# cv3vpl-lab/cylinder-pose-estimation

Measured on AMD Instinct MI355X. Metric: frames/sec (grid-detect + cylinder fit) on 1920x1200 batch, higher is better.
Workload: dtype f64

## Files before the change

### cylinder-pose-estimation_amd/csrc/ccl.hip

```cpp
#include "cpe_dev.h"

namespace cpe {

namespace {

__device__ __forceinline__ bool pred(const uint8_t *img, size_t i, int thr, int invert)
{
    return (((int)img[i] > thr) ? 1 : 0) != invert;
}

constexpr int CCL_INIT_ROWS = 16;
__global__ __launch_bounds__(256) void k_ccl_init(const uint8_t *__restrict__ img, int rows_total, int h, int w,
                                                  int thr, int invert, const FrameState *__restrict__ st, Window win,
                                                  int *__restrict__ L, int *__restrict__ cnt, CclOutside outside)
{
    const int lane = threadIdx.x & 63;
    for (int rr = 0; rr < CCL_INIT_ROWS / 4; rr++) {
    const int row = (blockIdx.x * (CCL_INIT_ROWS / 4) + rr) * 4 + (threadIdx.x >> 6);
    if (row >= rows_total) return;
    const int f = row / h, y = row - f * h;
    const Rect r = window_rect(st, f, win, h, w);
    if (y < r.y0 || y > r.y1 || r.x1 < r.x0) continue;
    const size_t base = (size_t)row * w;
    int carry_in = 0, carry_start = 0;
// ... 137 lines not shown
        const u64x2 *t = reinterpret_cast<const u64x2 *>(plane + bit_word(tc, y8, x0 >> 6));
#pragma unroll
        for (int q = 0; q < 4; q++) { const u64x2 v = t[q]; m[2 * q] = v.x; m[2 * q + 1] = v.y; }
    }
    __device__ __forceinline__ unsigned colbits(int y8, int ya, int yb, int x) const
    {
        unsigned long long m[CCL_STRIP];
        strip(y8, ya, yb, x & ~63, m);
        unsigned b = 0;
#pragma unroll
        for (int k = 0; k < CCL_STRIP; k++) b |= (unsigned)((m[k] >> (x & 63)) & 1ull) << k;
        return b;
    }
};

struct NotBitSrc {
    BitSrc b;
    size_t frame_words;
    __device__ __forceinline__ NotBitSrc frame(size_t f, int) const
    {
        return NotBitSrc{BitSrc{b.plane + f * frame_words, b.tc, b.plane_words}, frame_words};
    }
    __device__ __forceinline__ unsigned long long pack(int y, int x0) const { return ~b.pack(y, x0); }
    __device__ __forceinline__ bool px(int y, int x) const { return !b.px(y, x); }
    __device__ __forceinline__ void strip(int y8, int ya, int yb, int x0, unsigned long long (&m)[CCL_STRIP]) const
    {
        b.strip(y8, ya, yb, x0, m);
#pragma unroll
        for (int k = 0; k < CCL_STRIP; k++) m[k] = ~m[k];
    }
    __device__ __forceinline__ unsigned colbits(int y8, int ya, int yb, int x) const { return ~b.colbits(y8, ya, yb, x) & 0xffu; }
};

template <class SRC>
__global__ __launch_bounds__(256) void k_ccl_init64(SRC src0, int h, int w,
                                                    const FrameState *__restrict__ st, Window win, int *__restrict__ L)
{
    const int WW = (w + 63) >> 6, strips = (h + CCL_STRIP - 1) / CCL_STRIP;
    const size_t f = blockIdx.y;
    const int gi = blockIdx.x * 256 + threadIdx.x;
    if (gi >= WW * strips) return;
    const int sy = gi / WW, j = gi - sy * WW;
    const Rect r = window_rect(st, f, win, h, w);
    const int x0 = j * 64;
    if (r.x1 < r.x0 || x0 > r.x1 || x0 + 63 < r.x0) return;
    const int ya = max(sy * CCL_STRIP, r.y0), yb = min(sy * CCL_STRIP + CCL_STRIP - 1, r.y1);
    const size_t N = (size_t)h * w;
    const SRC src = src0.frame(f, h);
    int *Lf = L + f * N;
    const unsigned long long cmask = col_mask64(x0, r.x0, r.x1);
    const bool hasL = x0 - 1 >= r.x0;
    const int y8 = sy * CCL_STRIP;
    unsigned long long rows[CCL_STRIP], any = 0;
    src.strip(y8, ya, yb, x0, rows);
#pragma unroll
    for (int k = 0; k < CCL_STRIP; k++) any |= (y8 + k >= ya && y8 + k <= yb) ? rows[k] & cmask : 0ull;
    const unsigned lb = (hasL && (any & 1ull)) ? src.colbits(y8, ya, yb, x0 - 1) : 0u;
#pragma unroll
    for (int k = 0; k < CCL_STRIP; k++) {
        const int y = y8 + k;
        if (y < ya || y > yb) continue;
        unsigned long long m = rows[k] & cmask;
        if (!m) continue;
        const int base = y * w + x0;
        const bool cL = (m & 1ull) && ((lb >> k) & 1u);
        while (m) {
            const unsigned long long low = m & (0ull - m), run = m & ~(m + low);
            const int a = __ffsll((long long)low) - 1, e = a + __popcll(run);
            const int label = (a == 0 && cL) ? base - 1 : base + a;
            int b = a;
            while (b < e) {
                if ((b & 3) == 0 && b + 4 <= e) { *reinterpret_cast<int4 *>(Lf + base + b) = make_int4(label, label, label, label); b += 4; }
                else { Lf[base + b] = label; b++; }
            }
            m &= ~run;
        }
    }
}

template <class SRC>
__global__ __launch_bounds__(256) void k_ccl_merge64(SRC src0, int h, int w,
                                                     int conn8, const FrameState *__restrict__ st, Window win,
                                                     int *__restrict__ L)
{
    const int WW = (w + 63) >> 6, strips = (h + CCL_STRIP - 1) / CCL_STRIP;
    const size_t f = blockIdx.y;
    const int gi = blockIdx.x * 256 + threadIdx.x;
    if (gi >= WW * strips) return;
    const int sy = gi / WW, j = gi - sy * WW;
    const Rect r = window_rect(st, f, win, h, w);
    const int x0 = j * 64;
    if (r.x1 < r.x0 || x0 > r.x1 || x0 + 63 < r.x0) return;
    const int ya = max(sy * CCL_STRIP, r.y0 + 1), yb = min(sy * CCL_STRIP + CCL_STRIP - 1, r.y1);
    if (ya > yb) return;
    const size_t N = (size_t)h * w;
    const SRC src = src0.frame(f, h);
    int *Lf = L + f * N;
    const unsigned long long cmask = col_mask64(x0, r.x0, r.x1);
    const bool hasL = x0 - 1 >= r.x0, hasR = x0 + 64 <= r.x1;
    const int y8 = sy * CCL_STRIP;
    unsigned long long rows[CCL_STRIP], any = 0;
    src.strip(y8, ya - 1, yb, x0, rows);
#pragma unroll
    for (int k = 0; k < CCL_STRIP; k++) any |= (y8 + k >= ya - 1 && y8 + k <= yb) ? rows[k] & cmask : 0ull;
    const unsigned lb = (hasL && (any & 1ull)) ? src.colbits(y8, ya - 1, yb, x0 - 1) : 0u;
    const unsigned rb = (hasR && (any >> 63)) ? src.colbits(y8, ya - 1, yb, x0 + 64) : 0u;
    unsigned long long A = 0, aL = 0, aR = 0;
    if (ya == y8) {
        A = src.pack(ya - 1, x0) & cmask;
        aL = (hasL && src.px(ya - 1, x0 - 1)) ? 1ull : 0ull; aR = (hasR && src.px(ya - 1, x0 + 64)) ? 1ull : 0ull;
    }
#pragma unroll
    for (int k = 0; k < CCL_STRIP; k++) {
        const int y = y8 + k;
        if (y < ya - 1 || y > yb) continue;
        const unsigned long long C = rows[k] & cmask;
        const unsigned long long cL = (lb >> k) & 1u, cR = (rb >> k) & 1u;
        if (y == ya - 1) { A = C; aL = cL; aR = cR; continue; }
        if (C) {
            const unsigned long long Cs = (C << 1) | cL, As = (A << 1) | aL;
            const int base = y * w + x0;
            unsigned long long m = C & A & ~(Cs & As);
            while (m) { const int b = __ffsll((long long)m) - 1; m &= m - 1; uf_unite(Lf, base + b, base + b - w); }
            if (conn8) {
                const unsigned long long Cr = (C >> 1) | (cR << 63), Ar = (A >> 1) | (aR << 63);
                const unsigned long long nu = C & ~A;
                m = nu & Ar & ~Cr;
                while (m) { const int b = __ffsll((long long)m) - 1; m &= m - 1; uf_unite(Lf, base + b, base + b - w + 1); }
                m = nu & As & ~Cs;
                while (m) { const int b = __ffsll((long long)m) - 1; m &= m - 1; uf_unite(Lf, base + b, base + b - w - 1); }
            }
        }
        A = C; aL = cL; aR = cR;
    }
}

template <class SRC>
__global__ __launch_bounds__(256) void k_ccl_roots64(SRC src0, int h, int w,
                                                     FrameState *__restrict__ st, Window win, const int *__restrict__ L,
                                                     int *__restrict__ roots, RootList list)
{
    const int WW = (w + 63) >> 6, strips = (h + CCL_STRIP - 1) / CCL_STRIP;
    const size_t f = blockIdx.y;
    const int lane = threadIdx.x & 63;
    const int gi = blockIdx.x * 256 + threadIdx.x;
    const Rect r = window_rect(st, f, win, h, w);
    const size_t N = (size_t)h * w;
    const SRC src = src0.frame(f, h);
    const int *Lf = L + f * N;
    const int sy = gi / WW, j = gi - sy * WW, x0 = j * 64;
    const bool live = gi < WW * strips && !(r.x1 < r.x0 || x0 > r.x1 || x0 + 63 < r.x0);
    const int ya = live ? max(sy * CCL_STRIP, r.y0) : 0, yb = live ? min(sy * CCL_STRIP + CCL_STRIP - 1, r.y1) : -1;
    const unsigned long long cmask = live ? col_mask64(x0, r.x0, r.x1) : 0ull;
    const bool hasL = live && x0 - 1 >= r.x0;
    const int y8 = sy * CCL_STRIP;
    unsigned long long rows[CCL_STRIP], any = 0;
    unsigned lb = 0;
    if (live) {
        src.strip(y8, ya, yb, x0, rows);
#pragma unroll
        for (int k = 0; k < CCL_STRIP; k++) any |= (y8 + k >= ya && y8 + k <= yb) ? rows[k] & cmask : 0ull;
        if (hasL && (any & 1ull)) lb = src.colbits(y8, ya, yb, x0 - 1);
// ... 544 lines not shown
                if (__ballot(seed != cur)) {
                    o = flood_row(bg, seed, lane, WW);
                    if (lane < WW && o != cur) { out[(size_t)y * WW + lane] = o; any = true; }
                }
                prev = o;
            }
        }
        const int slot = ((pass + 1) >> 1) & 1;
        if (__ballot(any) && lane == 0) atomicOr(&s_any[slot], 1);
        __syncthreads();
        if (!upw) {
            const int ch = s_any[slot];
            __syncthreads();
            if (threadIdx.x == 0) s_any[slot] = 0;
            if (!ch) { converged = true; break; }
        }
    }
    if (!converged && threadIdx.x == 0) set_overflow(st[f], OVF_TRACE);
}

int outside_flood(const uint8_t *mask, int n, int h, int w, FrameState *st, Window win, unsigned long long *bgw,
                  unsigned long long *out, size_t plane_words, hipStream_t s, const uint32_t *bits)
{
    CPE_CHECK_ARG(w <= 4096 && plane_words >= (size_t)h * ((w + 63) >> 6), "outside_flood: frame too wide or scratch too small");
    CPE_LAUNCH_BEGIN();
    CPE_KLAUNCH(k_outside_flood, dim3(n), dim3(64 * FLOOD_BANDS), 0, s, mask, h, w, st, win, bgw, out, plane_words, bits);
    CPE_CHECK_LAUNCH("k_outside_flood");
    return CPE_OK;
}

static bool word_rows(const void *img, const int *L, int w) { return w % 16 == 0 && ((size_t)img & 15) == 0 && ((size_t)L & 15) == 0; }
static dim3 word_grid(int n, int h, int w) { return dim3((unsigned)((((w + 63) / 64) * ((h + CCL_STRIP - 1) / CCL_STRIP) + 255) / 256), n); }

static bool links8(const uint8_t *img, int n, int h, int w, int thr, Window win, int *L, FrameState *st, hipStream_t s)
{
    const size_t N = (size_t)h * w;
    if (word_rows(img, L, w)) {
        const ByteSrc src{img, w, thr, 0};
        CPE_KLAUNCH(k_ccl_init64<ByteSrc>, word_grid(n, h, w), dim3(256), 0, s, src, h, w, (const FrameState *)st, win, L);
        CPE_KLAUNCH(k_ccl_merge64<ByteSrc>, word_grid(n, h, w), dim3(256), 0, s, src, h, w, 1, (const FrameState *)st, win, L);
        return true;
    }
    CPE_KLAUNCH(k_ccl_init, dim3((n * h + CCL_INIT_ROWS - 1) / CCL_INIT_ROWS), dim3(256), 0, s, img, n * h, h, w, thr, 0, (const FrameState *)st, win, L,
                (int *)nullptr, OUTSIDE_UNTOUCHED);
    CPE_KLAUNCH(k_ccl_merge, dim3((unsigned)((N + CCL_BLK_PX - 1) / CCL_BLK_PX), n), dim3(256), 0, s, img, h, w, thr, 0, 1, (const FrameState *)st, win, L);
    return false;
}

bool ccl_components_reads_bits(const uint32_t *bits, int w, const int *L) { return bits && w % 16 == 0 && ((size_t)L & 15) == 0; }

int ccl_components(const uint8_t *img, const uint32_t *bits, int n, int h, int w, int thr, Window win, int *L, int *roots,
                   RootList list, FrameState *st, hipStream_t s)
{
    const size_t N = (size_t)h * w;
    const dim3 gw = word_grid(n, h, w);
    CPE_LAUNCH_BEGIN();
    CPE_KLAUNCH(k_ccl_ctl, dim3((n + 63) / 64), dim3(64), 0, s, st, (int *)nullptr, n, CTL_RESET_ROOTS, list);
    if (ccl_components_reads_bits(bits, w, L)) {
        const BitSrc src{bit_plane(bits, 0, h, w), bit_tile_cols(w), bit_plane_words(h, w)};
        CPE_KLAUNCH(k_ccl_init64<BitSrc>, gw, dim3(256), 0, s, src, h, w, (const FrameState *)st, win, L);
        CPE_KLAUNCH(k_ccl_merge64<BitSrc>, gw, dim3(256), 0, s, src, h, w, 1, (const FrameState *)st, win, L);
        CPE_KLAUNCH(k_ccl_roots64<BitSrc>, gw, dim3(256), 0, s, src, h, w, st, win, (const int *)L, roots, list);
    } else if (links8(img, n, h, w, thr, win, L, st, s)) {
        CPE_KLAUNCH(k_ccl_roots64<ByteSrc>, gw, dim3(256), 0, s, (ByteSrc{img, w, thr, 0}), h, w, st, win, (const int *)L, roots, list);
    } else {
        CPE_KLAUNCH(k_ccl_roots4, dim3((unsigned)((N + CCL_BLK_PX - 1) / CCL_BLK_PX), n), dim3(256), 0, s, img, h, w, thr, 0, st, win, (const int *)L,
                    roots, list);
    }
    CPE_CHECK_LAUNCH("ccl_components");
    return CPE_OK;
}

int ccl_unions(const uint8_t *mask, int n, int h, int w, Window win, int *L, FrameState *st, hipStream_t s)
{
    CPE_LAUNCH_BEGIN();
    links8(mask, n, h, w, 0, win, L, st, s);
    CPE_CHECK_LAUNCH("ccl_unions");
    return CPE_OK;
}

int ccl_label(const uint8_t *img, int n, int h, int w, int *L, const CclPass &p, FrameState *st, hipStream_t s)
{
    const size_t N = (size_t)h * w;
    CPE_LAUNCH_BEGIN();
    if (p.roots) CPE_KLAUNCH(k_ccl_ctl, dim3((n + 63) / 64), dim3(64), 0, s, st, (int *)nullptr, n, CTL_RESET_ROOTS, ROOTS_MAIN);
    CPE_KLAUNCH(k_ccl_init, dim3((n * h + CCL_INIT_ROWS - 1) / CCL_INIT_ROWS), dim3(256), 0, s, img, n * h, h, w, p.thr, p.invert, (const FrameState *)st, p.win, L,
                p.count ? p.cnt : (int *)nullptr, p.outside);
    if (word_rows(img, L, w))
        CPE_KLAUNCH(k_ccl_merge64<ByteSrc>, word_grid(n, h, w), dim3(256), 0, s, (ByteSrc{img, w, p.thr, p.invert}), h, w, p.conn8, (const FrameState *)st, p.win, L);
    else
        CPE_KLAUNCH(k_ccl_merge, dim3((unsigned)((N + CCL_BLK_PX - 1) / CCL_BLK_PX), n), dim3(256), 0, s, img, h, w, p.thr, p.invert, p.conn8,
                    (const FrameState *)st, p.win, L);
    if (p.touch) {
        (void)hipMemsetAsync(p.touch, 0, N * n, s);
        const int per = 2 * w + 2 * h;
        CPE_KLAUNCH(k_ccl_touch, dim3((n * per + 255) / 256), dim3(256), 0, s, (const int *)L, n, h, w, (const FrameState *)st, p.win, p.touch);
    }
    CPE_KLAUNCH(k_ccl_finish, dim3((unsigned)((N + CCL_FIN_PX - 1) / CCL_FIN_PX), n), dim3(256), 0, s, img, h, w, p.thr, p.invert, st, p.win, L,
                (const uint8_t *)p.touch, p.count, p.cnt, p.roots, p.nrect, p.outside, ROOTS_MAIN);
    CPE_CHECK_LAUNCH("ccl_label");
    return CPE_OK;
}

int ccl_dark_first(const uint8_t *img, const uint32_t *planes, int nplanes, int n, int h, int w, int thr, int *L, int *roots,
                   int *cnt, FrameState *st, hipStream_t s)
{
    if (!(word_rows(img, L, w) && planes && nplanes >= 1)) {
        CclPass p;
        p.thr = thr; p.invert = 1; p.conn8 = 0; p.win = WIN_SWEEP; p.outside = OUTSIDE_SWEEP_RUNS;
        p.count = COUNT_ALL; p.cnt = cnt; p.roots = roots;
        return ccl_label(img, n, h, w, L, p, st, s);
    }
    CPE_LAUNCH_BEGIN();
    CPE_KLAUNCH(k_ccl_ctl, dim3((n + 63) / 64), dim3(64), 0, s, st, (int *)nullptr, n, CTL_RESET_ROOTS, ROOTS_MAIN);
    CPE_KLAUNCH(k_ccl_init, dim3((n * h + CCL_INIT_ROWS - 1) / CCL_INIT_ROWS), dim3(256), 0, s, img, n * h, h, w, thr, 1, (const FrameState *)st, WIN_SWEEP, L,
                cnt, OUTSIDE_SWEEP_RUNS);
    const dim3 gw = word_grid(n, h, w);
    const NotBitSrc src{BitSrc{bit_plane(planes, 0, h, w), bit_tile_cols(w), bit_plane_words(h, w)}, (size_t)nplanes * bit_plane_words(h, w)};
    CPE_KLAUNCH(k_ccl_merge64<NotBitSrc>, gw, dim3(256), 0, s, src, h, w, 0, (const FrameState *)st, WIN_SWEEP, L);
    CPE_KLAUNCH(k_ccl_finish64<NotBitSrc>, gw, dim3(256), 0, s, src, h, w, st, WIN_SWEEP, L, cnt, roots, ROOTS_MAIN);
    CPE_CHECK_LAUNCH("ccl_dark_first");
    return CPE_OK;
}

int ccl_set_sweep_rect(FrameState *st, int *nrect, int n, hipStream_t s)
{
    CPE_LAUNCH_BEGIN();
    CPE_KLAUNCH(k_ccl_ctl, dim3((n + 63) / 64), dim3(64), 0, s, st, nrect, n, CTL_SWEEP_RECT, ROOTS_MAIN);
    CPE_CHECK_LAUNCH("k_ccl_ctl");
    return CPE_OK;
}

}
```

### cylinder-pose-estimation_amd/csrc/cpe_dev.h

```cpp
#pragma once
#include "cpe_internal.h"

namespace cpe {

constexpr int MAXROOTS = 262144;
enum { SWL_DARK = 0, SWL_BRIGHT = 1, SWL_TRACE = 2 };
__host__ __device__ inline int sweep_pool(int h, int w, int which)
{
    const long long N = (long long)h * w;
    long long v = which == SWL_TRACE ? N / 8 : N / 2;
    const long long lo = which == SWL_TRACE ? (1 << 18) : (1 << 19);
    v = v < lo ? lo : (v > (1 << 23) ? (1 << 23) : v);
    return (int)((v + 255) / 256 * 256);
}
constexpr int MAXJ = CPE_MAXJ;
constexpr int MAXB = 32768;
constexpr int MAXG = 32768;
constexpr int MAXG_LDS = 1024;
constexpr int GCAP = 48;
constexpr int MAXV = 131072;
constexpr int MAXL = CPE_MAXL;
constexpr int MAXLP = CPE_MAXLP;
constexpr int MAXSEG = 2048;

// ... 302 lines not shown
    }
    __device__ __forceinline__ void point(int x, int y, bool vertex)
    {
        npts++;
        if (vertex) nverts++;
        minx = min(minx, x); maxx = max(maxx, x); miny = min(miny, y); maxy = max(maxy, y);
        if (have_prev) edge(px, py, x, y);
        else { fx = x; fy = y; have_prev = true; }
        px = x; py = y;
    }
    __device__ __forceinline__ void finish() { if (have_prev) edge(px, py, fx, fy); }
    __device__ __forceinline__ bool stop() const { return false; }
};

__device__ __forceinline__ void moments_from_sums(long long a00, long long a10, long long a01, double &m00,
                                                  double &m10, double &m01)
{
    m00 = m10 = m01 = 0;
    double d00 = (double)a00;
    if (fabs(d00) > 1.1920928955078125e-07) {
        double db1_2, db1_6;
        if (d00 > 0) { db1_2 = 0.5; db1_6 = 0.16666666666666666666666666666667; }
        else { db1_2 = -0.5; db1_6 = -0.16666666666666666666666666666667; }
        m00 = d00 * db1_2;
        m10 = (double)a10 * db1_6;
        m01 = (double)a01 * db1_6;
    }
}

int build_bitplanes(const uint8_t *img, int n, int h, int w, int thr0, int step, int nplanes, uint32_t *planes, hipStream_t s);

int ccl_components(const uint8_t *img, const uint32_t *bits, int n, int h, int w, int thr, Window win, int *L, int *roots,
                   RootList list, FrameState *st, hipStream_t s);
bool ccl_components_reads_bits(const uint32_t *bits, int w, const int *L);
int ccl_unions(const uint8_t *mask, int n, int h, int w, Window win, int *L, FrameState *st, hipStream_t s);
int ccl_dark_first(const uint8_t *img, const uint32_t *planes, int nplanes, int n, int h, int w, int thr, int *L, int *roots,
                   int *cnt, FrameState *st, hipStream_t s);
enum CclOutside : int { OUTSIDE_NONE = 0, OUTSIDE_UNTOUCHED = 1, OUTSIDE_SWEEP_RUNS = 3 };
enum CclCount : int { COUNT_NONE = 0, COUNT_ALL = 1, COUNT_INTERIOR = 2, COUNT_ZERO = 3 };
struct CclPass {
    int thr = 0, invert = 0, conn8 = 1;
    Window win = WIN_FRAME;
    CclOutside outside = OUTSIDE_NONE;
    CclCount count = COUNT_NONE; int *cnt = nullptr;
    uint8_t *touch = nullptr;
    int *roots = nullptr;
    int *nrect = nullptr;
};
int ccl_label(const uint8_t *img, int n, int h, int w, int *L, const CclPass &p, FrameState *st, hipStream_t s);
int ccl_set_sweep_rect(FrameState *st, int *nrect, int n, hipStream_t s);

int outside_flood(const uint8_t *mask, int n, int h, int w, FrameState *st, Window win, unsigned long long *bgw,
                  unsigned long long *out, size_t plane_words, hipStream_t s, const uint32_t *bits);

int region_stage(const uint8_t *gray, int n, int h, int w, double clip, const RegionBuffers &B, FrameState *st, hipStream_t s,
                 const RegionSide *side, const uint8_t *lplane, const RegionProbe *probe);
int region_stage_plane(const uint8_t *gray, int n, int h, int w, const RegionBuffers &B, FrameState *st, hipStream_t s);
int region_hull(const uint8_t *img, int n, int h, int w, int thr, bool bits_ready, int single_is_positive, uint8_t *dst,
                const RegionBuffers &B, FrameState *st, hipStream_t s);
int clahe_front_probe(const uint8_t *gray, int n, int h, int w, int fused, int lab_lut, const RegionBuffers &B, hipStream_t s,
                      uint8_t *cl, uint32_t *planes, int *buckets, int *box);

int joints_mask_stage(int n, int h, int w, const MaskBuffers &B, FrameState *st, hipStream_t s);
int spot_stage(const uint8_t *gray, int n, int h, int w, const MaskBuffers &B, FrameState *st, hipStream_t s, int planar);
int masks_stage(const uint8_t *gray, int n, int h, int w, const MaskBuffers &B, FrameState *st, hipStream_t s,
                const RegionSide *side, int planar, hipStream_t sj);
// ... 14 lines not shown
```

### cylinder-pose-estimation_amd/csrc/detect.hip

```cpp
#include "workspace.h"
#include <ctype.h>
#include <mutex>
#include <stdlib.h>

namespace cpe {

namespace {

__global__ void k_state_init(FrameState *st, int n, unsigned long long *best, unsigned long long *best_s, int *nrect)
{
    int f = blockIdx.x * blockDim.x + threadIdx.x;
    if (f >= n) return;
    FrameState z = {};
    z.srect[0] = INT_MAX; z.srect[1] = INT_MAX; z.srect[2] = -1; z.srect[3] = -1;
    st[f] = z;
    if (best) { best[f] = 0; best_s[f] = 0; }
    if (nrect) { nrect[16 * f] = INT_MAX; nrect[16 * f + 1] = INT_MAX; nrect[16 * f + 2] = -1; nrect[16 * f + 3] = -1; }
}

__global__ void k_finish(const FrameState *st, int n, int *status, int *n_pts)
{
    int f = blockIdx.x * blockDim.x + threadIdx.x;
    if (f >= n) return;
    int s = st[f].status;
// ... 441 lines not shown
    CPE_CHECK_ARG(img && rect && ws && lab && cnt && roots && n_roots && n > 0 && h >= 64 && w >= 64 && (path == 0 || path == 1) &&
                  thr >= 0 && thr + 160 <= 255,
                  "cpe_debug_dark_labels: bad argument");
    Workspace W;
    if (int32_t rc = W.open(ws, ws_bytes, n, h, w, "cpe_debug_dark_labels")) return rc;
    hipStream_t s = (hipStream_t)stream;
    FrameState *st = W.state();
    int *lb = W.at<int>(WS_LABELS), *cb = W.at<int>(WS_LABELS_AUX), *rb = W.at<int>(WS_ROOTS);
    uint32_t *bits = W.at<uint32_t>(WS_BITS);
    const size_t N = (size_t)h * w;
    CPE_LAUNCH_BEGIN();
    CPE_KLAUNCH(k_state_init, dim3((n + 63) / 64), dim3(64), 0, s, st, n, (unsigned long long *)nullptr, (unsigned long long *)nullptr, (int *)nullptr);
    CPE_KLAUNCH(k_debug_rect, dim3((n + 63) / 64), dim3(64), 0, s, st, n, (const int *)rect);
    (void)hipMemsetAsync(lb, 0xff, N * n * sizeof(int), s);
    (void)hipMemsetAsync(cb, 0xff, N * n * sizeof(int), s);
    CPE_CHECK_LAUNCH("cpe_debug_dark_labels");
    int rc;
    if (path == 0) {
        CclPass p;
        p.thr = thr; p.invert = 1; p.conn8 = 0; p.win = WIN_SWEEP; p.outside = OUTSIDE_SWEEP_RUNS;
        p.count = COUNT_ALL; p.cnt = cb; p.roots = rb;
        rc = ccl_label(img, n, h, w, lb, p, st, s);
    } else if ((rc = build_bitplanes(img, n, h, w, thr, 10, 17, bits, s)) == CPE_OK)
        rc = ccl_dark_first(img, bits, 17, n, h, w, thr, lb, rb, cb, st, s);
    if (rc != CPE_OK) return rc;
    (void)hipMemcpyAsync(lab, lb, N * n * sizeof(int), hipMemcpyDeviceToDevice, s);
    (void)hipMemcpyAsync(cnt, cb, N * n * sizeof(int), hipMemcpyDeviceToDevice, s);
    (void)hipMemcpyAsync(roots, rb, (size_t)n * MAXROOTS * sizeof(int), hipMemcpyDeviceToDevice, s);
    CPE_KLAUNCH(k_debug_n_roots, dim3((n + 63) / 64), dim3(64), 0, s, (const FrameState *)st, n, n_roots);
    CPE_CHECK_LAUNCH("cpe_debug_dark_labels");
    return CPE_OK;
}

extern "C" int32_t cpe_debug_blob_region(const uint8_t *img, int32_t n, int32_t h, int32_t w, void *ws, size_t ws_bytes,
                                         float *kp, int32_t kp_cap, int32_t *n_kp, double *blobs, int32_t blob_cap,
                                         int32_t *n_blobs, void *stream)
{
    CPE_CHECK_ARG(img && ws && kp && n_kp && blobs && n_blobs && n > 0 && h >= 64 && w >= 64 && h <= 4096 && w <= 4096 &&
                  kp_cap > 0 && blob_cap > 0, "cpe_debug_blob_region: bad argument");
    Workspace W;
    if (int32_t rc = W.open(ws, ws_bytes, n, h, w, "cpe_debug_blob_region")) return rc;
    hipStream_t s = (hipStream_t)stream;
    FrameState *st = W.state();
    RegionBuffers R = region_buffers(W, h, w);
    RegionProbe probe = {1, blobs, blob_cap, n_blobs, kp, kp_cap, n_kp};
    CPE_LAUNCH_BEGIN();
    CPE_KLAUNCH(k_state_init, dim3((n + 63) / 64), dim3(64), 0, s, st, n, R.best, W.at<unsigned long long>(WS_BEST_SPOT), R.nrect);
    CPE_CHECK_LAUNCH("k_state_init");
    return region_stage(img, n, h, w, 4.5, R, st, s, nullptr, nullptr, &probe);
}

extern "C" int32_t cpe_debug_clahe_planes(const uint8_t *gray, int32_t n, int32_t h, int32_t w, int32_t fused, void *ws, size_t ws_bytes,
                                          uint8_t *cl, uint32_t *planes, int32_t *buckets, int32_t *box, void *stream)
{
    CPE_CHECK_ARG(gray && ws && cl && planes && buckets && box && n > 0 && h >= 64 && w >= 64 && h <= 4096 && w <= 4096,
                  "cpe_debug_clahe_planes: bad argument");
    Workspace W;
    if (int32_t rc = W.open(ws, ws_bytes, n, h, w, "cpe_debug_clahe_planes")) return rc;
    hipStream_t s = (hipStream_t)stream;
    FrameState *st = W.state();
    RegionBuffers R = region_buffers(W, h, w);
    CPE_LAUNCH_BEGIN();
    CPE_KLAUNCH(k_state_init, dim3((n + 63) / 64), dim3(64), 0, s, st, n, R.best, W.at<unsigned long long>(WS_BEST_SPOT), R.nrect);
    CPE_CHECK_LAUNCH("k_state_init");
    return clahe_front_probe(gray, n, h, w, fused, 1, R, s, cl, planes, buckets, box);
}
// ... 146 lines not shown
```

### cylinder-pose-estimation_amd/lib.py

```python
import ctypes as C
import os
import subprocess

_HERE = os.path.dirname(os.path.abspath(__file__))
SO_PATH = os.path.join(_HERE, 'libcpe_hip.so')
_lib = None


class CpeError(RuntimeError):
    pass


def build(verbose=False):
    cmd = ['make', '-C', os.path.join(_HERE, 'csrc'), '-j4']
    if not verbose:
        cmd.insert(1, '-s')
    subprocess.check_call(cmd)
    return SO_PATH


_SIGS = {
    'cpe_version': (C.c_int32, []),
    'cpe_last_error_string': (C.c_char_p, []),
    'cpe_profile_enable': (None, [C.c_int32]),
    'cpe_profile_report': (C.c_int32, [C.c_char_p, C.c_size_t]),
    'cpe_preprocess_batch': (C.c_int32, [C.c_void_p, C.c_int32, C.c_int32, C.c_int32, C.c_void_p, C.c_void_p]),
    'cpe_debug_preprocess': (C.c_int32, [C.c_void_p, C.c_int32, C.c_int32, C.c_int32] + [C.c_void_p] * 4),
    'cpe_detect_workspace_bytes': (C.c_size_t, [C.c_int32, C.c_int32, C.c_int32]),
    'cpe_detect_constants': (C.c_int32, [C.c_int32, C.c_void_p]),
    'cpe_detect_grid_batch': (C.c_int32, [C.c_void_p, C.c_int32, C.c_int32, C.c_int32, C.c_void_p, C.c_size_t] +
                              [C.c_void_p] * 6),
    'cpe_detect_grid_batch_ex': (C.c_int32, [C.c_void_p, C.c_int32, C.c_int32, C.c_int32, C.c_void_p, C.c_void_p, C.c_size_t] +
                                 [C.c_void_p] * 6),
    'cpe_detect_grid_bgr_batch_ex': (C.c_int32, [C.c_void_p, C.c_int32, C.c_int32, C.c_int32, C.c_void_p, C.c_void_p, C.c_size_t] +
                                     [C.c_void_p] * 6),
    'cpe_detect_line_tables': (C.c_int32, [C.c_void_p, C.c_size_t, C.c_int32, C.c_int32, C.c_int32, C.c_int32] + [C.c_void_p] * 5),
    'cpe_detect_results_sizes': (C.c_int32, [C.c_void_p, C.c_size_t, C.c_int32, C.c_int32, C.c_int32] + [C.c_void_p] * 4),
    'cpe_detect_results_pack': (C.c_int32, [C.c_void_p, C.c_size_t, C.c_int32, C.c_int32, C.c_int32] + [C.c_void_p] * 7 +
                                [C.c_size_t, C.c_void_p]),
    'cpe_bgr2gray_batch': (C.c_int32, [C.c_void_p, C.c_int32, C.c_int32, C.c_int32, C.c_void_p, C.c_void_p]),
    'cpe_detect_workspace_plane': (C.c_int32, [C.c_int32, C.c_int32, C.c_int32, C.c_int32, C.c_void_p, C.c_void_p]),
    'cpe_debug_workspace_buffer': (C.c_int32, [C.c_int32] * 4 + [C.c_char_p, C.c_size_t] + [C.c_void_p] * 5),
    'cpe_debug_external_components': (C.c_int32, [C.c_void_p, C.c_int32, C.c_int32, C.c_int32, C.c_void_p, C.c_size_t, C.c_void_p, C.c_int32,
                                                  C.c_void_p, C.c_void_p]),
    'cpe_debug_ccl': (C.c_int32, [C.c_void_p] + [C.c_int32] * 9 + [C.c_void_p, C.c_size_t, C.c_void_p]),
    'cpe_debug_dark_labels': (C.c_int32, [C.c_void_p] + [C.c_int32] * 4 + [C.c_void_p, C.c_int32, C.c_void_p, C.c_size_t] + [C.c_void_p] * 5),
    'cpe_debug_blob_region': (C.c_int32, [C.c_void_p] + [C.c_int32] * 3 + [C.c_void_p, C.c_size_t, C.c_void_p, C.c_int32, C.c_void_p,
                                                                           C.c_void_p, C.c_int32, C.c_void_p, C.c_void_p]),
    'cpe_debug_clahe_planes': (C.c_int32, [C.c_void_p] + [C.c_int32] * 4 + [C.c_void_p, C.c_size_t] + [C.c_void_p] * 5),
    'cpe_debug_clahe_planes_bgr': (C.c_int32, [C.c_void_p] + [C.c_int32] * 4 + [C.c_void_p, C.c_size_t] + [C.c_void_p] * 6),
    'cpe_debug_masks': (C.c_int32, [C.c_void_p] * 5 + [C.c_int32] * 4 + [C.c_void_p, C.c_size_t, C.c_void_p]),
    'cpe_debug_lines': (C.c_int32, [C.c_void_p] * 9 + [C.c_int32] * 3 + [C.c_void_p, C.c_void_p, C.c_size_t] + [C.c_void_p] * 6),
    'cpe_debug_region_hull': (C.c_int32, [C.c_void_p] + [C.c_int32] * 4 + [C.c_void_p, C.c_size_t, C.c_void_p]),
    'cpe_fit_workspace_bytes': (C.c_size_t, [C.c_int32]),
    'cpe_select_triangulate_batch': (C.c_int32, [C.c_void_p] * 6 + [C.c_int32] + [C.c_void_p] * 3 +
                                     [C.c_int32, C.c_int32, C.c_double, C.c_void_p, C.c_size_t] + [C.c_void_p] * 9),
    'cpe_choose_idx_batch': (C.c_int32, [C.c_void_p] * 6 + [C.c_int32] + [C.c_void_p] * 3 + [C.c_int32, C.c_double, C.c_void_p, C.c_size_t] +
                             [C.c_void_p] * 6),
    'cpe_triangulate_batch': (C.c_int32, [C.c_void_p] * 3 + [C.c_int32] + [C.c_void_p] * 7),
    'cpe_multi_frame_terms': (C.c_int32, [C.c_void_p, C.c_void_p, C.c_int32, C.c_void_p, C.c_void_p, C.c_double, C.c_void_p, C.c_void_p]),
    'cpe_multi_frame_fit_batch': (C.c_int32, [C.c_void_p] * 6 + [C.c_int32, C.c_int32, C.c_double, C.c_void_p] + [C.c_void_p] * 9),
    'cpe_multi_frame_fit_lm_batch': (C.c_int32, [C.c_void_p] * 6 + [C.c_int32, C.c_int32, C.c_double, C.c_void_p] + [C.c_void_p] * 10),
    'cpe_multi_frame_consensus_workspace_bytes': (C.c_size_t, [C.c_int32, C.c_int32]),
    'cpe_multi_frame_consensus_batch': (C.c_int32, [C.c_void_p] * 6 + [C.c_int32, C.c_int32, C.c_double, C.c_void_p, C.c_void_p, C.c_void_p,
                                                   C.c_size_t] + [C.c_void_p] * 13),
    'cpe_pose_vec2T_batch': (C.c_int32, [C.c_void_p, C.c_int32, C.c_void_p, C.c_void_p]),
    'cpe_pose_T2vec_batch': (C.c_int32, [C.c_void_p, C.c_int32, C.c_void_p, C.c_void_p]),
    'cpe_agv_chain_batch': (C.c_int32, [C.c_void_p, C.c_int32, C.c_void_p, C.c_void_p]),
    'cpe_frame_angles_lm_batch': (C.c_int32, [C.c_void_p] * 5 + [C.c_int32, C.c_int32, C.c_double, C.c_void_p] + [C.c_void_p] * 9),
    'cpe_fit_cylinder_ransac_batch': (C.c_int32, [C.c_void_p, C.c_void_p, C.c_int32, C.c_double, C.c_void_p, C.c_void_p] +
                                      [C.c_void_p] * 9),
    'cpe_match_offset_workspace_bytes': (C.c_size_t, [C.c_int32] * 3),
    'cpe_match_offset_batch': (C.c_int32, [C.c_void_p] * 6 + [C.c_int32] + [C.c_void_p] * 3 + [C.c_double, C.c_void_p, C.c_void_p, C.c_size_t] +
                               [C.c_void_p] * 6),
    'cpe_fit_plane_batch': (C.c_int32, [C.c_void_p] * 3 + [C.c_int32] + [C.c_void_p] * 10),
    'cpe_index_planes_batch': (C.c_int32, [C.c_void_p] * 3 + [C.c_int32, C.c_void_p, C.c_void_p, C.c_int32, C.c_int32, C.c_double] +
                               [C.c_void_p] * 8),
    'cpe_table_triangulate_batch': (C.c_int32, [C.c_void_p] * 3 + [C.c_int32] + [C.c_void_p] * 4 + [C.c_int32, C.c_int32] +
                                    [C.c_void_p] * 9),
# ... 153 lines not shown
```

### include/cpe.h

```cpp
#ifndef CPE_H
#define CPE_H

#include <stddef.h>
#include <stdint.h>

#ifdef __cplusplus
extern "C" {
#endif

#define CPE_VERSION 124

#if defined(__GNUC__)
#define CPE_API __attribute__((visibility("default")))
#else
#define CPE_API
#endif

#define CPE_OK 0
#define CPE_ERR_ARG (-1)
#define CPE_ERR_LAUNCH (-2)
#define CPE_ERR_WORKSPACE (-3)

#define CPE_ST_OK 0
#define CPE_ST_NO_REGION 1
#define CPE_ST_NO_SPOT 2
#define CPE_ST_NO_LINES 3
#define CPE_ST_EMPTY 4
#define CPE_ST_FEW_POINTS 5
#define CPE_ST_OVERFLOW 6
#define CPE_ST_SUBPIXEL_RAISED 7

CPE_API int32_t cpe_version(void);
CPE_API const char *cpe_last_error_string(void);

CPE_API void cpe_profile_enable(int32_t on);
CPE_API int32_t cpe_profile_report(char *csv, size_t cap);

CPE_API int32_t cpe_preprocess_batch(const uint8_t *gray, int32_t n, int32_t h, int32_t w, uint8_t *mask,
                             void *stream);

CPE_API int32_t cpe_debug_preprocess(const uint8_t *gray, int32_t n, int32_t h, int32_t w, uint8_t *mask, double *b,
                                     double *T, void *stream);

// ... 59 lines not shown
CPE_API int32_t cpe_bgr2gray_batch(const uint8_t *bgr, int32_t n, int32_t h, int32_t w, uint8_t *gray, void *stream);

#define CPE_PLANE_BINARY 0
#define CPE_PLANE_HMASK 1
#define CPE_PLANE_VMASK 2
#define CPE_PLANE_MASK_CONTOUR 3
#define CPE_PLANE_ROI_H 4
#define CPE_PLANE_ROI_V 5
#define CPE_PLANE_EXP_H 6
#define CPE_PLANE_EXP_V 7
#define CPE_PLANE_JOINTS 8
#define CPE_PLANE_STATE 9
#define CPE_PLANE_CLAHE 10
#define CPE_PLANE_BLUR19 11
#define CPE_PLANE_BLUR7 12
#define CPE_PLANE_SWEEP 14
CPE_API int32_t cpe_detect_workspace_plane(int32_t n, int32_t h, int32_t w, int32_t plane, size_t *offset,
                                           size_t *bytes_per_frame);

CPE_API int32_t cpe_debug_workspace_buffer(int32_t n, int32_t h, int32_t w, int32_t index, char *name_out, size_t name_cap,
                                           size_t *offset, size_t *bytes_per_frame, int32_t *overlay, int32_t *side,
                                           int32_t *public_plane);

#define CPE_PLANE_LABELS 13
CPE_API int32_t cpe_debug_ccl(const uint8_t *img, int32_t n, int32_t h, int32_t w, int32_t thr, int32_t invert,
                              int32_t conn8, int32_t count_mode, int32_t want_bbox, int32_t want_roots, void *ws,
                              size_t ws_bytes, void *stream);

#define CPE_MAXROOTS_DEBUG 262144
CPE_API int32_t cpe_debug_dark_labels(const uint8_t *img, int32_t n, int32_t h, int32_t w, int32_t thr, const int32_t *rect,
                                      int32_t path, void *ws, size_t ws_bytes, int32_t *lab, int32_t *cnt, int32_t *roots,
                                      int32_t *n_roots, void *stream);

CPE_API int32_t cpe_debug_external_components(const uint8_t *mask, int32_t n, int32_t h, int32_t w, void *ws, size_t ws_bytes,
                                              int32_t *first_px, int32_t cap, int32_t *count, void *stream);

CPE_API int32_t cpe_debug_clahe_planes(const uint8_t *gray, int32_t n, int32_t h, int32_t w, int32_t fused, void *ws, size_t ws_bytes,
                                       uint8_t *cl, uint32_t *planes, int32_t *buckets, int32_t *box, void *stream);

CPE_API int32_t cpe_debug_clahe_planes_bgr(const uint8_t *bgr, int32_t n, int32_t h, int32_t w, int32_t fused, void *ws,
                                           size_t ws_bytes, uint8_t *L, uint8_t *cl, uint32_t *planes, int32_t *buckets,
                                           int32_t *box, void *stream);

CPE_API int32_t cpe_debug_blob_region(const uint8_t *img, int32_t n, int32_t h, int32_t w, void *ws, size_t ws_bytes,
                                      float *kp, int32_t kp_cap, int32_t *n_kp, double *blobs, int32_t blob_cap,
                                      int32_t *n_blobs, void *stream);

CPE_API int32_t cpe_debug_masks(const uint8_t *binary, const uint8_t *gray, const uint8_t *mask_contour, const int32_t *rect,
                                const int32_t *region_status, int32_t n, int32_t h, int32_t w, int32_t target, void *ws,
                                size_t ws_bytes, void *stream);

CPE_API int32_t cpe_debug_lines(const uint8_t *exp_h, const uint8_t *exp_v, const int32_t *joints, const int32_t *n_joints,
                                const int32_t *rect, const int32_t *r0, const int32_t *stage_status, const uint8_t *g7,
                                const uint8_t *gray, int32_t n, int32_t h, int32_t w, const CpeDetectParams *params, void *ws,
                                size_t ws_bytes, double *xy, int32_t *id, int32_t *n_pts, double *center, int32_t *status,
                                void *stream);

CPE_API int32_t cpe_debug_region_hull(const uint8_t *img, int32_t n, int32_t h, int32_t w, int32_t mode, void *ws, size_t ws_bytes,
                                      void *stream);

#define CPE_MAXP 2048
#define CPE_FIT_TABLE_DIM 128

#define CPE_FIT_FLAG_FALLBACK 1
#define CPE_FIT_FLAG_OVERFLOW 2
#define CPE_FIT_MIN_POINTS 5
// ... 273 lines not shown
```

Measured before the change: 4106.

## Label whole 64x8 tile components locally in CCL init and skip intra-tile merges

The 64-bit word CCL init kernel now finds connected components inside each 64x8 tile with bitwise flood fill when the tile has few runs, and gives every pixel of a component the same label. The merge kernel can then skip vertical and diagonal union-find operations inside such tiles and only unites across tile edges, which reduces atomic union traffic. It adds register pressure and iterative fill loops in init, and adds a conn8 parameter plus a debug entry point.

```diff
diff --git a/cylinder-pose-estimation_amd/csrc/ccl.hip b/cylinder-pose-estimation_amd/csrc/ccl.hip
--- a/cylinder-pose-estimation_amd/csrc/ccl.hip
+++ b/cylinder-pose-estimation_amd/csrc/ccl.hip
@@ -193,8 +193,53 @@
     __device__ __forceinline__ unsigned colbits(int y8, int ya, int yb, int x) const { return ~b.colbits(y8, ya, yb, x) & 0xffu; }
 };
 
+
+__device__ __forceinline__ unsigned long long fill_runs(unsigned long long bg, unsigned long long f)
+{
+    f = (((bg + f) ^ bg) & bg) | f;
+    const unsigned long long rb = __brevll(bg), rf = __brevll(f);
+    return __brevll((((rb + rf) ^ rb) & rb) | rf);
+}
+__device__ __forceinline__ bool tile_spread(unsigned long long from, unsigned long long bg, unsigned long long &c, int conn8)
+{
+    unsigned long long s = conn8 ? (from | (from << 1) | (from >> 1)) : from;
+    s &= bg & ~c;
+    if (!s) return false;
+    c |= fill_runs(bg, s);
+    return true;
+}
+constexpr int CCL_TILE_RUNS = 24;
+__device__ __forceinline__ bool tile_is_local(const unsigned long long (&rows)[CCL_STRIP])
+{
+    int runs = 0;
+#pragma unroll
+    for (int k = 0; k < CCL_STRIP; k++) runs += __popcll(rows[k] & ~(rows[k] << 1));
+    return runs <= CCL_TILE_RUNS;
+}
+__device__ __forceinline__ unsigned row_mask8(int y8, int ya, int yb)
+{
+    return ya > yb ? 0u : (((2u << (yb - y8)) - 1u) & ~((1u << (ya - y8)) - 1u));
+}
+__device__ __forceinline__ void store_labels(int *Lrow, int a, int e, int label)
+{
+    int b = a;
+    while (b < e) {
+        if ((b & 3) == 0 && b + 4 <= e) { *reinterpret_cast<int4 *>(Lrow + b) = make_int4(label, label, label, label); b += 4; }
+        else { Lrow[b] = label; b++; }
+    }
+}
+__device__ __forceinline__ void store_row_labels(int *Lrow, unsigned long long m, int label)
+{
+    while (m) {
+        const unsigned long long low = m & (0ull - m), run = m & ~(m + low);
+        const int a = __ffsll((long long)low) - 1;
+        store_labels(Lrow, a, a + __popcll(run), label);
+        m &= ~run;
+    }
+}
+
 template <class SRC>
-__global__ __launch_bounds__(256) void k_ccl_init64(SRC src0, int h, int w,
+__global__ __launch_bounds__(256) void k_ccl_init64(SRC src0, int h, int w, int conn8,
                                                     const FrameState *__restrict__ st, Window win, int *__restrict__ L)
 {
     const int WW = (w + 63) >> 6, strips = (h + CCL_STRIP - 1) / CCL_STRIP;
@@ -215,31 +260,61 @@
     unsigned long long rows[CCL_STRIP], any = 0;
     src.strip(y8, ya, yb, x0, rows);
 #pragma unroll
-    for (int k = 0; k < CCL_STRIP; k++) any |= (y8 + k >= ya && y8 + k <= yb) ? rows[k] & cmask : 0ull;
+    for (int k = 0; k < CCL_STRIP; k++) { rows[k] = (y8 + k >= ya && y8 + k <= yb) ? rows[k] & cmask : 0ull; any |= rows[k]; }
+    if (!any) return;
     const unsigned lb = (hasL && (any & 1ull)) ? src.colbits(y8, ya, yb, x0 - 1) : 0u;
-#pragma unroll
-    for (int k = 0; k < CCL_STRIP; k++) {
-        const int y = y8 + k;
-        if (y < ya || y > yb) continue;
-        unsigned long long m = rows[k] & cmask;
-        if (!m) continue;
-        const int base = y * w + x0;
-        const bool cL = (m & 1ull) && ((lb >> k) & 1u);
-        while (m) {
-            const unsigned long long low = m & (0ull - m), run = m & ~(m + low);
-            const int a = __ffsll((long long)low) - 1, e = a + __popcll(run);
-            const int label = (a == 0 && cL) ? base - 1 : base + a;
-            int b = a;
-            while (b < e) {
-                if ((b & 3) == 0 && b + 4 <= e) { *reinterpret_cast<int4 *>(Lf + base + b) = make_int4(label, label, label, label); b += 4; }
-                else { Lf[base + b] = label; b++; }
-            }
-            m &= ~run;
-        }
-    }
-}
-
-template <class SRC>
+    if (!tile_is_local(rows)) {
+#pragma unroll
+        for (int k = 0; k < CCL_STRIP; k++) {
+            unsigned long long m = rows[k];
+            const int base = (y8 + k) * w + x0;
+            const bool cL = (m & 1ull) && ((lb >> k) & 1u);
+            while (m) {
+                const unsigned long long low = m & (0ull - m), run = m & ~(m + low);
+                const int a = __ffsll((long long)low) - 1;
+                store_labels(Lf + base, a, a + __popcll(run), (a == 0 && cL) ? base - 1 : base + a);
+                m &= ~run;
+            }
+        }
+        return;
+    }
+    for (;;) {
+        unsigned long long comp[CCL_STRIP];
+        int label = -1;
+#pragma unroll
+        for (int k = 0; k < CCL_STRIP; k++) {
+            comp[k] = 0ull;
+            if (label < 0 && rows[k]) {
+                const unsigned long long m = rows[k], low = m & (0ull - m);
+                const int base = (y8 + k) * w + x0;
+                comp[k] = m & ~(m + low);
+                label = ((low & 1ull) && ((lb >> k) & 1u)) ? base - 1 : base + __ffsll((long long)low) - 1;
+            }
+        }
+        if (label < 0) break;
+        for (bool down = true;; down = !down) {
+            bool grew = false;
+            if (down) {
+#pragma unroll
+                for (int k = 1; k < CCL_STRIP; k++) grew |= tile_spread(comp[k - 1], rows[k], comp[k], conn8);
+            } else {
+#pragma unroll
+                for (int k = CCL_STRIP - 2; k >= 0; k--) grew |= tile_spread(comp[k + 1], rows[k], comp[k], conn8);
+            }
+            if (!grew) break;
+        }
+#pragma unroll
+        for (int k = 0; k < CCL_STRIP; k++) rows[k] &= ~comp[k];
+        static_assert(CCL_STRIP == 8, "k_ccl_init64 stores the eight rows of a component one by one");
+        int *Lt = Lf + y8 * w + x0;
+        store_row_labels(Lt, comp[0], label);         store_row_labels(Lt + w, comp[1], label);
+        store_row_labels(Lt + 2 * w, comp[2], label); store_row_labels(Lt + 3 * w, comp[3], label);
+        store_row_labels(Lt + 4 * w, comp[4], label); store_row_labels(Lt + 5 * w, comp[5], label);
+        store_row_labels(Lt + 6 * w, comp[6], label); store_row_labels(Lt + 7 * w, comp[7], label);
+    }
+}
+
+template <class SRC, bool TILES>
 __global__ __launch_bounds__(256) void k_ccl_merge64(SRC src0, int h, int w,
                                                      int conn8, const FrameState *__restrict__ st, Window win,
                                                      int *__restrict__ L)
@@ -252,43 +327,46 @@
     const Rect r = window_rect(st, f, win, h, w);
     const int x0 = j * 64;
     if (r.x1 < r.x0 || x0 > r.x1 || x0 + 63 < r.x0) return;
-    const int ya = max(sy * CCL_STRIP, r.y0 + 1), yb = min(sy * CCL_STRIP + CCL_STRIP - 1, r.y1);
+    const int y8 = sy * CCL_STRIP;
+    const int ya = max(y8, r.y0), yb = min(y8 + CCL_STRIP - 1, r.y1);
     if (ya > yb) return;
     const size_t N = (size_t)h * w;
     const SRC src = src0.frame(f, h);
     int *Lf = L + f * N;
     const unsigned long long cmask = col_mask64(x0, r.x0, r.x1);
     const bool hasL = x0 - 1 >= r.x0, hasR = x0 + 64 <= r.x1;
-    const int y8 = sy * CCL_STRIP;
     unsigned long long rows[CCL_STRIP], any = 0;
-    src.strip(y8, ya - 1, yb, x0, rows);
-#pragma unroll
-    for (int k = 0; k < CCL_STRIP; k++) any |= (y8 + k >= ya - 1 && y8 + k <= yb) ? rows[k] & cmask : 0ull;
-    const unsigned lb = (hasL && (any & 1ull)) ? src.colbits(y8, ya - 1, yb, x0 - 1) : 0u;
-    const unsigned rb = (hasR && (any >> 63)) ? src.colbits(y8, ya - 1, yb, x0 + 64) : 0u;
+    src.strip(y8, ya, yb, x0, rows);
+#pragma unroll
+    for (int k = 0; k < CCL_STRIP; k++) { rows[k] = (y8 + k >= ya && y8 + k <= yb) ? rows[k] & cmask : 0ull; any |= rows[k]; }
+    if (!any) return;
+    const unsigned rm = row_mask8(y8, ya, yb);
+    const unsigned lb = (hasL && (any & 1ull)) ? src.colbits(y8, ya, yb, x0 - 1) & rm : 0u;
+    const unsigned rb = (hasR && (any >> 63)) ? src.colbits(y8, ya, yb, x0 + 64) & rm : 0u;
     unsigned long long A = 0, aL = 0, aR = 0;
-    if (ya == y8) {
-        A = src.pack(ya - 1, x0) & cmask;
-        aL = (hasL && src.px(ya - 1, x0 - 1)) ? 1ull : 0ull; aR = (hasR && src.px(ya - 1, x0 + 64)) ? 1ull : 0ull;
-    }
+    if (y8 - 1 >= r.y0 && rows[0]) {
+        A = src.pack(y8 - 1, x0) & cmask;
+        aL = (hasL && (rows[0] & 1ull) && src.px(y8 - 1, x0 - 1)) ? 1ull : 0ull;
+        aR = (hasR && (rows[0] >> 63) && src.px(y8 - 1, x0 + 64)) ? 1ull : 0ull;
+    }
+    const bool local = TILES && tile_is_local(rows);
 #pragma unroll
     for (int k = 0; k < CCL_STRIP; k++) {
-        const int y = y8 + k;
-        if (y < ya - 1 || y > yb) continue;
-        const unsigned long long C = rows[k] & cmask;
+        const unsigned long long C = rows[k];
         const unsigned long long cL = (lb >> k) & 1u, cR = (rb >> k) & 1u;
-        if (y == ya - 1) { A = C; aL = cL; aR = cR; continue; }
         if (C) {
+            const bool edges = local && k > 0;
             const unsigned long long Cs = (C << 1) | cL, As = (A << 1) | aL;
-            const int base = y * w + x0;
-            unsigned long long m = C & A & ~(Cs & As);
+            const int base = (y8 + k) * w + x0;
+            unsigned long long m = edges ? 0ull : C & A & ~(Cs & As);
             while (m) { const int b = __ffsll((long long)m) - 1; m &= m - 1; uf_unite(Lf, base + b, base + b - w); }
+            if (local && (C & 1ull) && cL && !(k > 0 && (A & 1ull) && aL) && uf_load(Lf, base) != base - 1) uf_unite(Lf, base, base - 1);
             if (conn8) {
                 const unsigned long long Cr = (C >> 1) | (cR << 63), Ar = (A >> 1) | (aR << 63);
                 const unsigned long long nu = C & ~A;
-                m = nu & Ar & ~Cr;
+                m = nu & Ar & ~Cr & (edges ? 1ull << 63 : ~0ull);
                 while (m) { const int b = __ffsll((long long)m) - 1; m &= m - 1; uf_unite(Lf, base + b, base + b - w + 1); }
-                m = nu & As & ~Cs;
+                m = nu & As & ~Cs & (edges ? 1ull : ~0ull);
                 while (m) { const int b = __ffsll((long long)m) - 1; m &= m - 1; uf_unite(Lf, base + b, base + b - w - 1); }
             }
         }
@@ -899,18 +977,18 @@
 static bool word_rows(const void *img, const int *L, int w) { return w % 16 == 0 && ((size_t)img & 15) == 0 && ((size_t)L & 15) == 0; }
 static dim3 word_grid(int n, int h, int w) { return dim3((unsigned)((((w + 63) / 64) * ((h + CCL_STRIP - 1) / CCL_STRIP) + 255) / 256), n); }
 
-static bool links8(const uint8_t *img, int n, int h, int w, int thr, Window win, int *L, FrameState *st, hipStream_t s)
+static bool links(const uint8_t *img, int n, int h, int w, int thr, int conn8, Window win, int *L, FrameState *st, hipStream_t s)
 {
     const size_t N = (size_t)h * w;
     if (word_rows(img, L, w)) {
         const ByteSrc src{img, w, thr, 0};
-        CPE_KLAUNCH(k_ccl_init64<ByteSrc>, word_grid(n, h, w), dim3(256), 0, s, src, h, w, (const FrameState *)st, win, L);
-        CPE_KLAUNCH(k_ccl_merge64<ByteSrc>, word_grid(n, h, w), dim3(256), 0, s, src, h, w, 1, (const FrameState *)st, win, L);
+        CPE_KLAUNCH(k_ccl_init64<ByteSrc>, word_grid(n, h, w), dim3(256), 0, s, src, h, w, conn8, (const FrameState *)st, win, L);
+        CPE_KLAUNCH((k_ccl_merge64<ByteSrc, true>), word_grid(n, h, w), dim3(256), 0, s, src, h, w, conn8, (const FrameState *)st, win, L);
         return true;
     }
     CPE_KLAUNCH(k_ccl_init, dim3((n * h + CCL_INIT_ROWS - 1) / CCL_INIT_ROWS), dim3(256), 0, s, img, n * h, h, w, thr, 0, (const FrameState *)st, win, L,
                 (int *)nullptr, OUTSIDE_UNTOUCHED);
-    CPE_KLAUNCH(k_ccl_merge, dim3((unsigned)((N + CCL_BLK_PX - 1) / CCL_BLK_PX), n), dim3(256), 0, s, img, h, w, thr, 0, 1, (const FrameState *)st, win, L);
+    CPE_KLAUNCH(k_ccl_merge, dim3((unsigned)((N + CCL_BLK_PX - 1) / CCL_BLK_PX), n), dim3(256), 0, s, img, h, w, thr, 0, conn8, (const FrameState *)st, win, L);
     return false;
 }
 
@@ -918,6 +996,12 @@
 
 int ccl_components(const uint8_t *img, const uint32_t *bits, int n, int h, int w, int thr, Window win, int *L, int *roots,
                    RootList list, FrameState *st, hipStream_t s)
+{
+    return ccl_components_conn(img, bits, n, h, w, thr, 1, win, L, roots, list, st, s);
+}
+
+int ccl_components_conn(const uint8_t *img, const uint32_t *bits, int n, int h, int w, int thr, int conn8, Window win, int *L,
+                        int *roots, RootList list, FrameState *st, hipStream_t s)
 {
     const size_t N = (size_t)h * w;
     const dim3 gw = word_grid(n, h, w);
@@ -925,10 +1009,10 @@
     CPE_KLAUNCH(k_ccl_ctl, dim3((n + 63) / 64), dim3(64), 0, s, st, (int *)nullptr, n, CTL_RESET_ROOTS, list);
     if (ccl_components_reads_bits(bits, w, L)) {
         const BitSrc src{bit_plane(bits, 0, h, w), bit_tile_cols(w), bit_plane_words(h, w)};
-        CPE_KLAUNCH(k_ccl_init64<BitSrc>, gw, dim3(256), 0, s, src, h, w, (const FrameState *)st, win, L);
-        CPE_KLAUNCH(k_ccl_merge64<BitSrc>, gw, dim3(256), 0, s, src, h, w, 1, (const FrameState *)st, win, L);
+        CPE_KLAUNCH(k_ccl_init64<BitSrc>, gw, dim3(256), 0, s, src, h, w, conn8, (const FrameState *)st, win, L);
+        CPE_KLAUNCH((k_ccl_merge64<BitSrc, true>), gw, dim3(256), 0, s, src, h, w, conn8, (const FrameState *)st, win, L);
         CPE_KLAUNCH(k_ccl_roots64<BitSrc>, gw, dim3(256), 0, s, src, h, w, st, win, (const int *)L, roots, list);
-    } else if (links8(img, n, h, w, thr, win, L, st, s)) {
+    } else if (links(img, n, h, w, thr, conn8, win, L, st, s)) {
         CPE_KLAUNCH(k_ccl_roots64<ByteSrc>, gw, dim3(256), 0, s, (ByteSrc{img, w, thr, 0}), h, w, st, win, (const int *)L, roots, list);
     } else {
         CPE_KLAUNCH(k_ccl_roots4, dim3((unsigned)((N + CCL_BLK_PX - 1) / CCL_BLK_PX), n), dim3(256), 0, s, img, h, w, thr, 0, st, win, (const int *)L,
@@ -941,7 +1025,7 @@
 int ccl_unions(const uint8_t *mask, int n, int h, int w, Window win, int *L, FrameState *st, hipStream_t s)
 {
     CPE_LAUNCH_BEGIN();
-    links8(mask, n, h, w, 0, win, L, st, s);
+    links(mask, n, h, w, 0, 1, win, L, st, s);
     CPE_CHECK_LAUNCH("ccl_unions");
     return CPE_OK;
 }
@@ -954,7 +1038,7 @@
     CPE_KLAUNCH(k_ccl_init, dim3((n * h + CCL_INIT_ROWS - 1) / CCL_INIT_ROWS), dim3(256), 0, s, img, n * h, h, w, p.thr, p.invert, (const FrameState *)st, p.win, L,
                 p.count ? p.cnt : (int *)nullptr, p.outside);
     if (word_rows(img, L, w))
-        CPE_KLAUNCH(k_ccl_merge64<ByteSrc>, word_grid(n, h, w), dim3(256), 0, s, (ByteSrc{img, w, p.thr, p.invert}), h, w, p.conn8, (const FrameState *)st, p.win, L);
+        CPE_KLAUNCH((k_ccl_merge64<ByteSrc, false>), word_grid(n, h, w), dim3(256), 0, s, (ByteSrc{img, w, p.thr, p.invert}), h, w, p.conn8, (const FrameState *)st, p.win, L);
     else
         CPE_KLAUNCH(k_ccl_merge, dim3((unsigned)((N + CCL_BLK_PX - 1) / CCL_BLK_PX), n), dim3(256), 0, s, img, h, w, p.thr, p.invert, p.conn8,
                     (const FrameState *)st, p.win, L);
@@ -984,7 +1068,7 @@
                 cnt, OUTSIDE_SWEEP_RUNS);
     const dim3 gw = word_grid(n, h, w);
     const NotBitSrc src{BitSrc{bit_plane(planes, 0, h, w), bit_tile_cols(w), bit_plane_words(h, w)}, (size_t)nplanes * bit_plane_words(h, w)};
-    CPE_KLAUNCH(k_ccl_merge64<NotBitSrc>, gw, dim3(256), 0, s, src, h, w, 0, (const FrameState *)st, WIN_SWEEP, L);
+    CPE_KLAUNCH((k_ccl_merge64<NotBitSrc, false>), gw, dim3(256), 0, s, src, h, w, 0, (const FrameState *)st, WIN_SWEEP, L);
     CPE_KLAUNCH(k_ccl_finish64<NotBitSrc>, gw, dim3(256), 0, s, src, h, w, st, WIN_SWEEP, L, cnt, roots, ROOTS_MAIN);
     CPE_CHECK_LAUNCH("ccl_dark_first");
     return CPE_OK;
diff --git a/cylinder-pose-estimation_amd/csrc/cpe_dev.h b/cylinder-pose-estimation_amd/csrc/cpe_dev.h
--- a/cylinder-pose-estimation_amd/csrc/cpe_dev.h
+++ b/cylinder-pose-estimation_amd/csrc/cpe_dev.h
@@ -358,6 +358,8 @@
 
 int ccl_components(const uint8_t *img, const uint32_t *bits, int n, int h, int w, int thr, Window win, int *L, int *roots,
                    RootList list, FrameState *st, hipStream_t s);
+int ccl_components_conn(const uint8_t *img, const uint32_t *bits, int n, int h, int w, int thr, int conn8, Window win, int *L,
+                        int *roots, RootList list, FrameState *st, hipStream_t s);
 bool ccl_components_reads_bits(const uint32_t *bits, int w, const int *L);
 int ccl_unions(const uint8_t *mask, int n, int h, int w, Window win, int *L, FrameState *st, hipStream_t s);
 int ccl_dark_first(const uint8_t *img, const uint32_t *planes, int nplanes, int n, int h, int w, int thr, int *L, int *roots,
diff --git a/cylinder-pose-estimation_amd/csrc/detect.hip b/cylinder-pose-estimation_amd/csrc/detect.hip
--- a/cylinder-pose-estimation_amd/csrc/detect.hip
+++ b/cylinder-pose-estimation_amd/csrc/detect.hip
@@ -497,6 +497,35 @@
     return CPE_OK;
 }
 
+extern "C" int32_t cpe_debug_ccl_tiles(const uint8_t *img, int32_t n, int32_t h, int32_t w, int32_t thr, int32_t conn8,
+                                       int32_t bits, const int32_t *rect, void *ws, size_t ws_bytes, int32_t *lab, int32_t *roots,
+                                       int32_t *n_roots, void *stream)
+{
+    CPE_CHECK_ARG(img && ws && lab && roots && n_roots && n > 0 && h >= 1 && w >= 16 && thr >= 0 && thr <= 255,
+                  "cpe_debug_ccl_tiles: bad argument");
+    Workspace W;
+    if (int32_t rc = W.open(ws, ws_bytes, n, h, w, "cpe_debug_ccl_tiles")) return rc;
+    hipStream_t s = (hipStream_t)stream;
+    FrameState *st = W.state();
+    int *lb = W.at<int>(WS_LABELS), *rb = W.at<int>(WS_ROOTS);
+    uint32_t *planes = W.at<uint32_t>(WS_BITS);
+    const size_t N = (size_t)h * w;
+    CPE_LAUNCH_BEGIN();
+    CPE_KLAUNCH(k_state_init, dim3((n + 63) / 64), dim3(64), 0, s, st, n, (unsigned long long *)nullptr, (unsigned long long *)nullptr, (int *)nullptr);
+    if (rect) CPE_KLAUNCH(k_debug_rect, dim3((n + 63) / 64), dim3(64), 0, s, st, n, (const int *)rect);
+    (void)hipMemsetAsync(lb, 0xff, N * n * sizeof(int), s);
+    CPE_CHECK_LAUNCH("cpe_debug_ccl_tiles");
+    int rc;
+    if (bits && (rc = build_bitplanes(img, n, h, w, thr, 0, 1, planes, s)) != CPE_OK) return rc;
+    if ((rc = ccl_components_conn(img, bits ? planes : nullptr, n, h, w, thr, conn8 ? 1 : 0, rect ? WIN_SWEEP : WIN_FRAME, lb, rb, ROOTS_MAIN,
+                                  st, s)) != CPE_OK) return rc;
+    (void)hipMemcpyAsync(lab, lb, N * n * sizeof(int), hipMemcpyDeviceToDevice, s);
+    (void)hipMemcpyAsync(roots, rb, (size_t)n * MAXROOTS * sizeof(int), hipMemcpyDeviceToDevice, s);
+    CPE_KLAUNCH(k_debug_n_roots, dim3((n + 63) / 64), dim3(64), 0, s, (const FrameState *)st, n, n_roots);
+    CPE_CHECK_LAUNCH("cpe_debug_ccl_tiles");
+    return CPE_OK;
+}
+
 extern "C" int32_t cpe_debug_blob_region(const uint8_t *img, int32_t n, int32_t h, int32_t w, void *ws, size_t ws_bytes,
                                          float *kp, int32_t kp_cap, int32_t *n_kp, double *blobs, int32_t blob_cap,
                                          int32_t *n_blobs, void *stream)
diff --git a/cylinder-pose-estimation_amd/lib.py b/cylinder-pose-estimation_amd/lib.py
--- a/cylinder-pose-estimation_amd/lib.py
+++ b/cylinder-pose-estimation_amd/lib.py
@@ -45,6 +45,7 @@
                                                   C.c_void_p, C.c_void_p]),
     'cpe_debug_ccl': (C.c_int32, [C.c_void_p] + [C.c_int32] * 9 + [C.c_void_p, C.c_size_t, C.c_void_p]),
     'cpe_debug_dark_labels': (C.c_int32, [C.c_void_p] + [C.c_int32] * 4 + [C.c_void_p, C.c_int32, C.c_void_p, C.c_size_t] + [C.c_void_p] * 5),
+    'cpe_debug_ccl_tiles': (C.c_int32, [C.c_void_p] + [C.c_int32] * 6 + [C.c_void_p, C.c_void_p, C.c_size_t] + [C.c_void_p] * 4),
     'cpe_debug_blob_region': (C.c_int32, [C.c_void_p] + [C.c_int32] * 3 + [C.c_void_p, C.c_size_t, C.c_void_p, C.c_int32, C.c_void_p,
                                                                            C.c_void_p, C.c_int32, C.c_void_p, C.c_void_p]),
     'cpe_debug_clahe_planes': (C.c_int32, [C.c_void_p] + [C.c_int32] * 4 + [C.c_void_p, C.c_size_t] + [C.c_void_p] * 5),
diff --git a/include/cpe.h b/include/cpe.h
--- a/include/cpe.h
+++ b/include/cpe.h
@@ -8,7 +8,7 @@
 extern "C" {
 #endif
 
-#define CPE_VERSION 124
+#define CPE_VERSION 125
 
 #if defined(__GNUC__)
 #define CPE_API __attribute__((visibility("default")))
@@ -134,6 +134,10 @@
                                       int32_t path, void *ws, size_t ws_bytes, int32_t *lab, int32_t *cnt, int32_t *roots,
                                       int32_t *n_roots, void *stream);
 
+CPE_API int32_t cpe_debug_ccl_tiles(const uint8_t *img, int32_t n, int32_t h, int32_t w, int32_t thr, int32_t conn8,
+                                    int32_t bits, const int32_t *rect, void *ws, size_t ws_bytes, int32_t *lab, int32_t *roots,
+                                    int32_t *n_roots, void *stream);
+
 CPE_API int32_t cpe_debug_external_components(const uint8_t *mask, int32_t n, int32_t h, int32_t w, void *ws, size_t ws_bytes,
                                               int32_t *first_px, int32_t cap, int32_t *count, void *stream);
 
```

Result: faster. 4169 (median of 6 runs) (+1.5%).
